# ishine/usdm

Measured on AMD Instinct MI355X. Metric: end-to-end real-time factor + LLM tokens/sec, 10 s utterance, 7B TP=1/8, higher is better.
Workload: dtype bf16; 1 GPU; full pipeline, one 10 s utterance: XLS-R tokenizer -> Mistral-7B (3 greedy rounds) -> Token-Voicebox 63 NFE (Heun, CFG, 3 s prompt) -> BigVGAN; wave_samples=160000, mel_frames=861, output_samples=220416, parallelism=tp1 (LLM) + replicas, tp_comm=none, voicebox=replica (CFG batch 2 on every rank)

## Files before the change

include/usdm_hip.h:

```cpp
#ifndef USDM_HIP_H_
#define USDM_HIP_H_
#include <stdint.h>

#ifdef __cplusplus
extern "C" {
#endif

typedef void* usdm_stream_t;

enum { USDM_BF16 = 0, USDM_F32 = 1 };
enum { USDM_ACT_NONE = 0, USDM_ACT_GELU = 1, USDM_ACT_SWIGLU = 3, USDM_ACT_TANH = 4, USDM_ACT_LOGCLAMP = 5  };
enum { USDM_EPI_PLAIN = 0, USDM_EPI_QKV_HEADS = 1 };

const char* usdm_last_error(void);
int usdm_abi_version(void);

typedef struct usdm_gemm_args {
  int32_t dtype;
  int32_t M, N;
  int32_t taps, Kc;
  const void* A;
  int64_t lda;
  int32_t rowsA;
  int32_t a_row_mul, a_row_off, a_row_step;
// ... 143 lines not shown
int64_t usdm_gemv_batch_ks_floats(int32_t N, int32_t K);
int usdm_gemv_batch(const usdm_gemv_batch_args* args, usdm_stream_t stream);

typedef struct usdm_gemv_fp8_args {
  usdm_gemv_batch_args b;
  const int8_t* row_exp;
} usdm_gemv_fp8_args;
int usdm_gemv_fp8(const usdm_gemv_fp8_args* args, usdm_stream_t stream);
int usdm_gemv_fp8_mfma(const usdm_gemv_fp8_args* args, usdm_stream_t stream);
int usdm_dequant_fp8(const void* q, const int8_t* row_exp, int32_t N, int32_t K, int64_t ldq, void* out, int64_t ldo,
                     usdm_stream_t stream);
int usdm_sizeof_gemv_fp8_args(void);

typedef struct usdm_gemv_mxfp4_args {
  usdm_gemv_batch_args b;
  const uint8_t* scales;
  int64_t lds;
} usdm_gemv_mxfp4_args;
int usdm_gemv_mxfp4(const usdm_gemv_mxfp4_args* args, usdm_stream_t stream);
int usdm_dequant_mxfp4(const void* codes, int64_t ldw, const uint8_t* scales, int64_t lds, int32_t N, int32_t K, void* out,
                       int64_t ldo, usdm_stream_t stream);
int usdm_sizeof_gemv_mxfp4_args(void);

typedef struct usdm_decode_state {
  int32_t* next_token;
  int32_t* out_tokens;
  int32_t* step;
  int32_t* pos;
  int32_t max_out, id_offset, advance_pos;
  int32_t batch;
  int32_t* done; const int32_t* eos;
} usdm_decode_state;
int usdm_argmax_final(const float* part_val, const int32_t* part_idx, int32_t nparts,
                      const usdm_decode_state* st, const void* embed_table_bf16, int32_t Hd, void* h_out_bf16,
                      usdm_stream_t stream);
int usdm_argmax_final_seg(const float* part_val, const int32_t* part_idx, int32_t nparts, int32_t nseg, int64_t seg_stride,
                          const usdm_decode_state* st, const void* embed_table, int32_t Hd, void* h_out, usdm_stream_t stream);

typedef struct usdm_sample_params {
  float temperature; int32_t top_k; float top_p;
  float min_p;
  uint64_t seed;
} usdm_sample_params;
typedef struct usdm_sample_args {
  const float* logits; int32_t V;
  float temperature; int32_t top_k; float top_p;
// ... 243 lines not shown
```

usdm_amd/_lib.py:

```python
import ctypes as C
import os

_HERE = os.path.dirname(os.path.abspath(__file__))
LIB_PATH = os.path.join(_HERE, "libusdm_hip.so")


class UsdmError(RuntimeError):
    pass


if not os.path.exists(LIB_PATH):
    raise ImportError(
        f"{LIB_PATH} not found: build it with `python -m usdm_amd.build` (hipcc --offload-arch=gfx950). "
        "usdm_amd has no CPU fallback.")

lib = C.CDLL(LIB_PATH, mode=C.RTLD_GLOBAL)
lib.usdm_last_error.restype = C.c_char_p
lib.usdm_gemv_batch_ks_floats.restype = C.c_int64
lib.usdm_gemv_fp8_mfma.restype = C.c_int
lib.usdm_attn_decode_fp8.restype = C.c_int
lib.usdm_rope_cache_fp8.restype = C.c_int
lib.usdm_gemv_mxfp4.restype = C.c_int
lib.usdm_dequant_mxfp4.restype = C.c_int
lib.usdm_logprobs.restype = C.c_int
lib.usdm_logprobs_seg.restype = C.c_int
lib.usdm_prompt_logprobs.restype = C.c_int
lib.usdm_prompt_logprobs_seg.restype = C.c_int
lib.usdm_penalize.restype = C.c_int
lib.usdm_penalize_seg.restype = C.c_int
lib.usdm_penalty_params_init.restype = C.c_int
lib.usdm_logit_edit.restype = C.c_int
lib.usdm_logit_edit_seg.restype = C.c_int
lib.usdm_beam_step.restype = C.c_int
lib.usdm_kv_reorder.restype = C.c_int
lib.usdm_kv_expand.restype = C.c_int
lib.usdm_attn_verify.restype = C.c_int
lib.usdm_spec_commit.restype = C.c_int
lib.usdm_attn_verify_batch.restype = C.c_int
lib.usdm_spec_commit_batch.restype = C.c_int
_exp = None


def exp():
    global _exp
    if _exp is None:
        path = os.path.join(_HERE, "libusdm_hip_experimental.so")
# ... 302 lines not shown
```

usdm_amd/csrc/gemv_common.h:

```cpp
#pragma once
#include "common.h"
#include "../../include/usdm_hip.h"

#ifndef USDM_UNR1
#define USDM_UNR1 8
#endif

namespace {
typedef __attribute__((ext_vector_type(2))) __bf16 bf16x2;

__device__ __forceinline__ float dot8(u32x4 w, u32x4 x, float acc) {
#pragma unroll
  for (int i = 0; i < 4; ++i) {
    const unsigned a = w[i], b = x[i];
    acc = __builtin_amdgcn_fdot2_f32_bf16(__builtin_bit_cast(bf16x2, a), __builtin_bit_cast(bf16x2, b), acc, false);
  }
  return acc;
}

template <bool FP8> struct gemv_fmt { typedef u32x4 wvec; };
template <> struct gemv_fmt<true> { typedef u32x2 wvec; };
struct gemv_mx4 { const uint8_t* scales; int64_t lds; };
template <class... FMT> struct gemv_is_mx4 { static constexpr bool value = false; };
template <> struct gemv_is_mx4<gemv_mx4> { static constexpr bool value = true; };
template <int I> struct gemv_ic { static constexpr int value = I; };
__device__ __forceinline__ const int8_t* gemv_row_exp() { return nullptr; }
__device__ __forceinline__ const int8_t* gemv_row_exp(const int8_t* e) { return e; }
__device__ __forceinline__ gemv_mx4 gemv_mx4_fmt() { return gemv_mx4{nullptr, 0}; }
__device__ __forceinline__ gemv_mx4 gemv_mx4_fmt(const int8_t*) { return gemv_mx4{nullptr, 0}; }
__device__ __forceinline__ gemv_mx4 gemv_mx4_fmt(gemv_mx4 m) { return m; }
constexpr int gemv_ring_depth(int NR, bool FP8, bool MX4) {
  const int bf16_depth = NR >= 8 ? 2 : NR >= 4 ? 4 : NR == 3 ? 5 : NR == 2 ? 8 : USDM_UNR1;
  return MX4 ? (NR >= 3 ? 2 : 4) : FP8 ? 2 * bf16_depth : bf16_depth;
}

__device__ __forceinline__ float gemv_sumsq8(u32x4 v, float ss) {
#pragma unroll
  for (int e = 0; e < 4; ++e) {
    const float lo = bf2f(v[e] & 0xffff), hi = bf2f(v[e] >> 16);
    ss += lo * lo + hi * hi;
  }
  return ss;
}
__device__ __forceinline__ u32x4 gemv_rmsnorm8(u32x4 v, float rstd, float4 g0, float4 g1) {
  const float gw[8] = {g0.x, g0.y, g0.z, g0.w, g1.x, g1.y, g1.z, g1.w};
  u32x4 o;
#pragma unroll
  for (int e = 0; e < 4; ++e) {
    const float lo = bf2f(v[e] & 0xffff), hi = bf2f(v[e] >> 16);
    o[e] = pack_bf2(round_bf(round_bf(lo * rstd) * gw[2 * e]), round_bf(round_bf(hi * rstd) * gw[2 * e + 1]));
  }
  return o;
}
__device__ __forceinline__ int gemv_glu_row(int o, bool up) { return (o >> 4) * 32 + (o & 15) + (up ? 16 : 0); }
__device__ __forceinline__ float gemv_swiglu_value(float g, float u, bool round_bf16) {
  if (round_bf16) {
// ... 17 lines not shown
```

usdm_amd/csrc/gemv_pieces.h:

```cpp
#pragma once
#include "gemv_common.h"

namespace {
__device__ __forceinline__ void gemv_load16(u32x4& dst, const void* p) {
  asm volatile("global_load_dwordx4 %0, %1, off" : "=v"(dst) : "v"(p) : "memory");
}
__device__ __forceinline__ void gemv_early_loads(const usdm_gemv_args& a, int i0, int K, u32x4& x0, u32x4& ge0v, u32x4& ge1v) {
  const int ic = min(i0, K - 8);
  const float* gp0 = a.norm_w ? a.norm_w + ic : (const float*)a.x;
  const float* gp1 = a.norm_w ? gp0 + 4 : gp0;
  gemv_load16(x0, (const bf16_t*)a.x + ic);
  gemv_load16(ge0v, gp0);
  gemv_load16(ge1v, gp1);
}
template <int IT>
__device__ __forceinline__ void gemv_ring_load(u32x4& dst, const char* row, unsigned voff) {
  const unsigned vo = voff + (IT >> 2) * 4096u;
  asm volatile("global_load_dwordx4 %0, %1, %2 offset:%3 nt" : "=v"(dst) : "v"(vo), "s"(row), "n"((IT & 3) * 1024) : "memory");
}

template <int NWV>
__device__ __forceinline__ float gemv_rms_rstd(float ss, float* red, int K, float eps) {
  const int lane = threadIdx.x & 63, wave = threadIdx.x >> 6;
  ss = wave_sum(ss);
  if (lane == 0) red[wave] = ss;
  __syncthreads();
  float tot = 0.f;
#pragma unroll
  for (int w = 0; w < NWV; ++w) tot += red[w];
  return rsqrtf(tot / (float)K + eps);
}
}
```

usdm_amd/csrc/llm_k.hip:

```cpp
#include "common.h"
#include <stdlib.h>
#include <utility>
#include "../../include/usdm_hip.h"
#include "gemv_launch.h"
#include "gemv_pieces.h"
#include "attn_merge.h"
#include "p2p.h"
#include "pick_commit.h"

#ifndef USDM_GEMV_DOWN_UNR
#define USDM_GEMV_DOWN_UNR 8
#endif
namespace {
#ifdef USDM_GEMV_TRACE
__device__ unsigned long long g_gemv_trace[8192 * 8];
#define GTR(i) do { if (threadIdx.x == 0 && blockIdx.x < 8192) g_gemv_trace[blockIdx.x * 8 + (i)] = wall_clock64(); } while (0)
#else
#define GTR(i) do { } while (0)
#endif


template <int RW, bool GLU, int NWV, bool MRG = false, bool P2P = false, bool CMB = false, bool FP8 = false, class... FMT>
__global__ __launch_bounds__(NWV * 64) void gemv_kernel(const usdm_gemv_args a, FMT... fmt) {
  typedef typename gemv_fmt<FP8>::wvec wvec;
  constexpr bool MX4 = gemv_is_mx4<FMT...>::value;
  static_assert((FP8 || MX4) == (sizeof...(FMT) == 1) && !(FP8 && MX4), "FP8 takes the row exponents, MXFP4 the block scales");
  static_assert(!(FP8 || MX4) || (!MRG && !P2P && !CMB), "the FP8 / MXFP4 weight formats have the plain single-GPU forms only");
  constexpr int NTH = NWV * 64;
  constexpr int NR = GLU ? 2 * RW : RW;
  constexpr int UNR = gemv_ring_depth(NR, FP8, MX4);
  extern __shared__ __attribute__((aligned(16))) char smem[];
  bf16_t* xs = (bf16_t*)smem;
  __shared__ float red[NWV];
  __shared__ float sv[NWV];
// ... 528 lines not shown
  __syncthreads();
  GTR(2);

  float acc = 0.f;
  u32x4 xv = *(const u32x4*)(xs + lane * 8);
  gemv_for<NIT>([&](auto IT) {
    constexpr int it = decltype(IT)::value, u = it % UNR;
    constexpr int younger = it + UNR < NIT ? UNR - 1 : NIT - 1 - it;
    const u32x4 xn = *(const u32x4*)(xs + (((it + 1) % NIT) * 64 + lane) * 8);
    asm volatile("s_waitcnt vmcnt(%1)" : "+v"(ring[u]) : "n"(younger) : "memory");
    acc = dot8(ring[u], xv, acc);
    if constexpr (it + UNR < NIT) gemv_ring_load<it + UNR>(ring[u], wp, voff);
    xv = xn;
  });
  acc = wave_sum(acc);
  GTR(3);

  if (lane != 0 || ob >= a.N) return;
  const float v = gemv_plain_value(acc, a.round_bf16, a.residual != nullptr, [&] { return bf2f(resraw); });
  if (a.y16) ((bf16_t*)a.y16)[ob] = f2bf(v);
  if (a.y32) a.y32[ob] = v;
}

__global__ void argmax_final_kernel(const float* pv, const int* pi, int nparts, int nseg, int64_t seg_stride, usdm_decode_state st,
                                    const bf16_t* E, int Hd, bf16_t* h_out) {
  __shared__ float sv[256];
  __shared__ int si[256];
  __shared__ int s_tok;
  const int b = blockIdx.x;
  if (st.done && st.done[b]) return;
  pv += (int64_t)b * nparts; pi += (int64_t)b * nparts;
  float bv = -INFINITY;
  int bi = PICK_NO_ID;
  for (int sg = 0; sg < nseg; ++sg)
    for (int i = threadIdx.x; i < nparts; i += 256) {
      const float v = pv[sg * seg_stride + i];
      const int id = pi[sg * seg_stride + i];
      if (pick_better(v, id, bv, bi)) { bv = v; bi = id; }
    }
  pick_block_best<256>(sv, si, bv, bi);
  if (threadIdx.x == 0) {
    const int tok = (si[0] == PICK_NO_ID ? 0 : si[0]) + st.id_offset;
    pick_commit(st, b, st.step[b], tok);
    s_tok = tok;
  }
  if (E) {
// ... 93 lines not shown
  USDM_CHECK_ARG(!a.x_out || (a.x_delta && a.x_out != a.x), "usdm_gemv: x_out needs x_delta and must not alias x");
  USDM_CHECK_ARG(!a.mrg_po || (a.mrg_pm && a.mrg_pl && a.mrg_ns >= 1 && a.mrg_ns <= 64 && a.K % 128 == 0 && !a.norm_w && !a.x_delta),
                 "usdm_gemv: merged-attention input needs pm/pl/po, 1 <= splits <= 64, K a multiple of 128, no norm / x_delta");
  USDM_CHECK_ARG(a.p2p_mode >= 0 && a.p2p_mode <= 2, "usdm_gemv: p2p_mode");
  USDM_CHECK_ARG(!a.p2p_mode || (a.p2p && a.p2p_site >= 0 && a.act == USDM_ACT_NONE && !a.part_val && a.residual && a.y16),
                 "usdm_gemv: the fused all-reduce needs a plain row-parallel projection with residual + y16");
  const int nout = glu ? a.N / 2 : a.N;
  hipStream_t st = (hipStream_t)stream;
  if (a.cmb_gran) {
    USDM_CHECK_ARG(a.mrg_po && a.mrg_pm && a.mrg_pl && a.mrg_ns >= 1 && a.mrg_ns <= 64 && !a.p2p_mode && !glu && !a.part_val && !a.norm_w && !a.x_delta &&
                       nout % 256 == 0 && nout / 256 == 16 && a.K % 128 == 0 && a.K / 128 <= 256,
                   "usdm_gemv: cmb_gran needs the mrg_* partials, a plain 4096-output projection and K / 128 <= 256 heads");
    return gemv_launch<GEMV_CMB, false, false, true, false>(a, st);
  }
  if (a.mrg_po || a.p2p_mode) {
    USDM_CHECK_ARG(!glu && !a.part_val, "usdm_gemv: merged-attention input / fused all-reduce are for plain projections");
    if (a.mrg_po && a.p2p_mode) return gemv_launch<GEMV_MRG, true, true, false, false>(a, st);
    if (a.mrg_po) return gemv_launch<GEMV_MRG, true, false, false, false>(a, st);
    return gemv_launch<GEMV_MRG, false, true, false, false>(a, st);
  }
  return gemv_launch<GEMV_PLAIN, false, false, false, false>(a, st);
}

int usdm_gemv_fp8_batch_launch(const usdm_gemv_fp8_args* pa, hipStream_t st);

extern "C" int usdm_gemv_fp8(const usdm_gemv_fp8_args* pa, usdm_stream_t stream) {
  USDM_CHECK_ARG(pa && pa->b.g.W && pa->b.g.x && pa->row_exp, "usdm_gemv_fp8: null args");
  const usdm_gemv_args& a = pa->b.g;
  USDM_CHECK_ARG(pa->b.nb >= 1 && pa->b.nb <= 4 && (pa->b.form == 0 || pa->b.form == -1),
                 "usdm_gemv_fp8: 1..4 sequences on the VALU form (the matrix-core form has no FP8 weights)");
  USDM_CHECK_ARG(!a.p2p && !a.p2p_mode && !a.mrg_po && !a.cmb_gran && !a.x_delta && !a.x_out,
                 "usdm_gemv_fp8: p2p / merged-attention input / cmb_gran / x_delta are not supported with FP8 weights");
  USDM_CHECK_ARG(((uintptr_t)a.W & 7) == 0, "usdm_gemv_fp8: bad N/K/ldw");
  if (int rc = gemv_check_shape("usdm_gemv_fp8", a, "input vector")) return rc;
  if (int rc = gemv_check_outputs("usdm_gemv_fp8", a)) return rc;
  hipStream_t st = (hipStream_t)stream;
  if (pa->b.nb > 1) return usdm_gemv_fp8_batch_launch(pa, st);
  return gemv_launch<GEMV_PLAIN, false, false, false, true>(a, st, pa->row_exp);
}

namespace {
__global__ __launch_bounds__(256) void dequant_fp8_kernel(const uint8_t* q, const int8_t* row_exp, int K, int64_t ldq, bf16_t* out,
                                                          int64_t ldo) {
  const int r = blockIdx.x;
  const float s = fp8_row_scale(row_exp[r]);
  const uint8_t* qr = q + (int64_t)r * ldq;
// ... 126 lines not shown
```

usdm_amd/llm.py:

```python
import math
import os
from collections import namedtuple

import torch

from . import ops
from ._lib import ACT_SWIGLU
from .graph import GraphedPlan, GraphedSegments
from .plancache import LRU
from .prefix import reusable_past
from .quant import Fp8Weight, Mxfp4Weight, check_kv_cache_dtype
from .slots import (CHUNK, NO_CANDIDATE_IDX, BeamSlots, DecodeSlots, SpecSequence, SpecSlots, TokenLogprobs, edit_buffers, logprob_buffers,
                    penalty_buffers, read_logprobs, seed_edits, seed_penalties, stop_block, stop_index)

MISTRAL_7B_USDM = dict(vocab_size=42003, hidden_size=4096, intermediate_size=14336, num_hidden_layers=32,
                       num_attention_heads=32, num_key_value_heads=8, head_dim=128, rms_norm_eps=1e-5,
                       rope_theta=10000.0, max_position_embeddings=32768)


def _pack_gate_up(gate, up):
    I, K = gate.shape
    return torch.stack([gate.reshape(I // 16, 16, K), up.reshape(I // 16, 16, K)], 1).reshape(2 * I, K).contiguous()


def vocab_shard(V, rank, tp):
    Vloc = (V + tp - 1) // tp
    v0 = min(V, rank * Vloc)
    v1 = min(V, v0 + Vloc)
    return Vloc, v0, v1, ops.gemv_nblocks(Vloc)


def agree_seed(seed, group, rank, device=None):
    import torch.distributed as dist
    if hasattr(group, "usdm_all_gather"):
# ... 122 lines not shown
    g = lambda n: sd_get(n).to(device, dtype)
    f = lambda n: sd_get(n).to(device, torch.float32).contiguous()
    W = {"embed": g("model.embed_tokens.weight").contiguous(), "norm": f("model.norm.weight"),
         "lm_head": qz_head(g("lm_head.weight")[v0:v1].contiguous()), "layers": [], "v0": v0, "v1": v1}
    for l in range(cfg["num_hidden_layers"]):
        p = f"model.layers.{l}."
        q = g(p + "self_attn.q_proj.weight")[rank * Hq * d:(rank + 1) * Hq * d]
        k = g(p + "self_attn.k_proj.weight")[rank * Hkv * d:(rank + 1) * Hkv * d]
        v = g(p + "self_attn.v_proj.weight")[rank * Hkv * d:(rank + 1) * Hkv * d]
        o = g(p + "self_attn.o_proj.weight")[:, rank * Hq * d:(rank + 1) * Hq * d]
        ga = g(p + "mlp.gate_proj.weight")[rank * I:(rank + 1) * I]
        up = g(p + "mlp.up_proj.weight")[rank * I:(rank + 1) * I]
        dn = g(p + "mlp.down_proj.weight")[:, rank * I:(rank + 1) * I]
        W["layers"].append(dict(qkv=qz(torch.cat([q, k, v], 0).contiguous()), o=qz(o.contiguous()), gu=qz(_pack_gate_up(ga, up)),
                                down=qz(dn.contiguous()), ln1=f(p + "input_layernorm.weight"),
                                ln2=f(p + "post_attention_layernorm.weight")))
        del q, k, v, o, ga, up, dn
    return W


class USDMForCausalLM:
    def __init__(self, cfg, device, ctx_max=2048, tp_rank=0, tp_size=1, group=None, decode_splits=None, tp_segments=None, p2p=None,
                 p2p_fused=None, quantization=None, fp8_matrix_cores=False, kv_cache_dtype=None, score_rows=256,
                 enable_prefix_caching=False):
        check_quantization(quantization, fp8_matrix_cores)
        self.prefix_caching = bool(enable_prefix_caching)
        if self.prefix_caching:
            if tp_size > 1 or tp_segments or p2p is not None:
                raise NotImplementedError("enable_prefix_caching runs on one GPU: tensor parallelism (tp_size > 1, tp_segments, p2p) is not supported")
            if os.environ.get("USDM_PREFIX_REUSE", "exact") in ("0", "off"):
                raise ValueError("enable_prefix_caching=True contradicts USDM_PREFIX_REUSE=0 (prefix reuse switched off)")
        if isinstance(score_rows, bool) or not isinstance(score_rows, int) or score_rows < 16 or score_rows % 16:
            raise ValueError(f"score_rows must be a positive multiple of 16, got {score_rows!r}")
        self.score_rows = score_rows
        if quantization is not None and (tp_size > 1 or tp_segments or p2p is not None):
            raise NotImplementedError(f"quantization={quantization!r} runs on one GPU: tensor parallelism (tp_size > 1, tp_segments, p2p) takes bf16 weights")
        self.kv_cache_dtype = check_kv_cache_dtype(kv_cache_dtype)
        self.kv8 = self.kv_cache_dtype == "fp8"
        if self.kv8 and (tp_size > 1 or tp_segments or p2p is not None):
            raise NotImplementedError("kv_cache_dtype='fp8' runs on one GPU: tensor parallelism (tp_size > 1, tp_segments, p2p) takes a bf16 cache")
        if self.kv8 and os.environ.get("USDM_GEMV_CHAIN", "0") not in ("", "0"):
            raise NotImplementedError("kv_cache_dtype='fp8': the chained decode GEMVs (USDM_GEMV_CHAIN) take a bf16 cache")
        self.quantization = quantization
        self.fp8_matrix_cores = bool(fp8_matrix_cores)
        self.cfg = dict(cfg)
        self.device = torch.device(device)
        if self.device.type != "cuda":
            raise RuntimeError("USDMForCausalLM (usdm_amd) runs on the MI355X only; there is no CPU fallback")
# ... 123 lines not shown
                           p + "self_attn.o_proj.weight": ((H, c["num_attention_heads"] * d), H ** -0.5),
                           p + "mlp.gate_proj.weight": ((I, H), H ** -0.5), p + "mlp.up_proj.weight": ((I, H), H ** -0.5),
                           p + "mlp.down_proj.weight": ((H, I), I ** -0.5)})

        def get(n):
            if n.endswith("norm.weight") or n.endswith("layernorm.weight"):
                return torch.ones(H, device=m.device)
            shape, sc = shapes[n]
            return (torch.randn(shape, device=m.device, dtype=torch.float32, generator=gen) * sc).to(torch.bfloat16)
        m.W = m._shard(get)
        m._alloc()
        return m

    def weight_bytes_per_token(self):
        if self.quantization is not None:
            return sum(l[k].nbytes for l in self.W["layers"] for k in QUANT_KEYS) + self.W["lm_head"].nbytes
        n = sum(l[k].numel() for l in self.W["layers"] for k in ("qkv", "o", "gu", "down")) + self.W["lm_head"].numel()
        return 2 * n

    def kv_bytes_per_token_row(self):
        d = self.cfg["head_dim"]
        return 2 * self.cfg["num_hidden_layers"] * self.Hkv * ((d + 1) if self.kv8 else 2 * d)

    def _alloc(self):
        c, dev = self.cfg, self.device
        L, d = c["num_hidden_layers"], c["head_dim"]
        bf = torch.bfloat16
        if self.kv8:
            self.kcache = torch.zeros(L, self.Hkv, self.ctx_max, d, dtype=torch.uint8, device=dev)
            self.vcache = torch.zeros(L, self.Hkv, self.ctx_max, d, dtype=torch.uint8, device=dev)
            self.kexp = torch.zeros(L, self.Hkv, self.ctx_max, dtype=torch.int8, device=dev)
            self.vexp = torch.zeros(L, self.Hkv, self.ctx_max, dtype=torch.int8, device=dev)
        else:
            self.kcache = torch.zeros(L, self.Hkv, self.ctx_max, d, dtype=bf, device=dev)
            self.vcache = torch.zeros(L, self.Hkv, self.ctx_max, d, dtype=bf, device=dev)
        mode = os.environ.get("USDM_PREFIX_REUSE", "exact")
        self.reuse_prefix = {"0": False, "off": False, "1": True, "all": True}.get(mode, "exact")
        if self.kv8:
            self.vtc = None
            if not self.prefix_caching:
                self.reuse_prefix = False
        else:
            self.vtc = torch.zeros(L, self.Hkv, d, self.ctx_max, dtype=bf, device=dev)
        self._kv_ids, self._vt_upto = None, 0
        inv_freq = 1.0 / (c["rope_theta"] ** (torch.arange(0, d, 2, dtype=torch.int64).float() / d))
        fr = torch.arange(self.ctx_max).float()[:, None] * inv_freq[None, :]
        self.cos = fr.cos().to(bf).to(dev).contiguous()
# ... 146 lines not shown
                ops.penalize(logits, st, V=self.v1 - self.v0, plan=rec.plan, **pen)
            if sampling == "hook":
                rec.cut(lambda: self.logits_hook())
            ops.sample_final(logits, st, dev_params=sl.sample_params, plan=rec.plan, **out)
            if lp:
                ops.logprobs(logits, st, V=self.v1 - self.v0, plan=rec.plan, **lp)
        elif p2p is not None:
            site = 2 * c["num_hidden_layers"]
            self._p2p_exchange(rec, st, lambda ph: ops.argmax_p2p(sl.part_val_loc, sl.part_idx_loc, self.nparts, st, p2p, site, phase=ph,
                                                                  plan=rec.plan, **out))
        else:
            if self.tp_path:
                rec.cut(self._gather_partials if single else
                        (lambda: self._gather_partials([sl.part_val, sl.part_idx], [sl.part_val_loc, sl.part_idx_loc])))
            seg = dict(nseg=self.tp_size, seg_stride=B * self.nparts) if (B and self.tp_path) else {}
            ops.argmax_final(sl.part_val, sl.part_idx, self.nparts * (1 if B else self.tp_size), st, plan=rec.plan, **seg, **out)
        rec.plan.hold(st)

    def _dims(self):
        c = self.cfg
        H, d = c["hidden_size"], c["head_dim"]
        return H, d, c["num_hidden_layers"], self.Hq, self.Hkv, self.I, (self.Hq + 2 * self.Hkv) * d

    def _layers(self, rec, gemv, attn, h, qkv, ao, act, way, n=0, parts=None, h_alt=None, down_kw={}):
        H, d, _, Hq, Hkv, I, nq = self._dims()
        eps, h0, pend = self.cfg["rms_norm_eps"], h, None

        def proj(W, ln, N, out, a=0):
            nonlocal h, pend
            if pend is None:
                return gemv(W, h, N=N, K=H, norm_w=ln, eps=eps, act=a, y16=out)
            nxt = h_alt if h is h0 else h0
            gemv(W, h, N=N, K=H, norm_w=ln, eps=eps, act=a, y16=out, x_delta=pend, x_out=nxt)
            h, pend = nxt, None

        def land(W, x, K, site, **kw):
            nonlocal pend
            if way == "fused":
                return gemv(W, x, N=H, K=K, residual=h, y16=h, **kw)
            if way == "p2p":
                mode = 1 if self.p2p_fused else 2
                gemv(W, x, N=H, K=K, residual=h, y16=h, p2p=self.p2p, p2p_site=site, p2p_mode=mode, **kw)
                rec.cut()
                if mode == 2:
                    ops.p2p_reduce(self.p2p, site, H, h, skip=self.st_done, plan=rec.plan)
                return
            part = parts[site & 1]
            gemv(W, x, N=H, K=K, round_bf16=False, y32=part, **kw)
            rec.cut(lambda: self._all_reduce(part))
            if way == "deferred":
                pend = part
            else:
                ops.residual_add(h, part, n, plan=rec.plan)

        for l, w in enumerate(self.W["layers"]):
            proj(w["qkv"], w["ln1"], nq, qkv)
            o_kw = attn(l) or {}
            land(w["o"], ao, Hq * d, 2 * l, **o_kw)
            proj(w["gu"], w["ln2"], 2 * I, act, ACT_SWIGLU)
            land(w["down"], act, I, 2 * l + 1, **down_kw)
        return h, pend

    def _prefill_rows(self, S, slot=None, past=0):
        dev, bf = self.device, torch.bfloat16
        H, d, L, Hq, Hkv, I, nq = self._dims()
        scratch = slot is not None or self.kv8
        Spad = ((past if scratch else 0) + S + 63) // 64 * 64
        rec = _Segments()
        Z = lambda *s, dt=bf: rec.plan.hold(torch.zeros(*s, device=dev, dtype=dt))
        io = dict(ids=Z(S, dt=torch.int64))
        h, xn, qkv, ao, act = Z(S, H), Z(S, H), Z(S, nq), Z(S, Hq * d), Z(S, I)
        vt = Z(Hkv, d, Spad) if scratch else None
        kscr = Z(Hkv, Spad, d) if self.kv8 else None
        part = Z(S, H, dt=torch.float32) if self.tp_path else None
        ops.embed_rows(self.W["embed"], h, Hd=H, ids=io["ids"], n=S, plan=rec.plan)

        def gemm(W, x, *, N, K, norm_w=None, eps=None, act=0, residual=None, y16=None, y32=None, round_bf16=True):
            if norm_w is not None:
                ops.norm(x, norm_w, None, rows=S, C=H, eps=eps, rms=True, round_bf16=True, out16=xn, plan=rec.plan)
                x = xn
            ops.gemm(x, self._gemm_w(W, rec.plan), M=S, N=N, Kc=K, act=act, round_bf16=round_bf16 and (bool(act) or residual is not None),
                     residual=residual, ldr=H if residual is not None else 0, out32=y32, out16=y16, ldc=N // 2 if act else N, plan=rec.plan)

# ... 95 lines not shown
                ops.gemv_engine(chain, sync, self.chain_gran, plan=rec.plan)
            else:
                ops.gemv_chain(chain, sync, plan=rec.plan)
            chain = None

        def gemv(W, x, **kw):
            if chain is None:
                return ops.gemv(W, x, skip=skp, plan=rec.plan, **kw)
            chain.append(ops.gemv(W, x, skip=skp, only_args=True, **kw))
            if len(chain) == self.chain:
                flush()

        def attn(l):
            nonlocal chain
            gran = cmb_gran[l] if use_cmb else None
            ops.attn_decode(qkv, self.st_pos, self.cos, self.sin, self.kcache[l], self.vcache[l], pm, pl, po, ao, Hq=Hq, Hkv=Hkv,
                            ctx_max=self.ctx_max, NS=self.NS, scale=d ** -0.5, counters=cnt, skip=skp, defer_merge=mrg is not None, window=self.window,
                            cmb_gran=gran, kv8=(self.kexp[l], self.vexp[l]) if self.kv8 else None, plan=rec.plan)
            if chained:
                chain = []
                return None
            return dict(merge=mrg, cmb=(gran, self.cmb_err) if use_cmb else None)

        h, pend = self._layers(rec, gemv, attn, h, qkv, ao, act, way, n=H, parts=parts, h_alt=h_alt)
        if chain:
            flush()
        self._lm_head_and_pick(rec, h, True, sampling, x_delta=pend, skip=skp, logprobs=logprobs, penalties=penalties, edits=edits)
        return rec.finish()

    @staticmethod
    def _run_segs(segs):
        for s in segs:
            if isinstance(s, ops.Plan):
                s.run()
            else:
                s()

    def _graphed(self, built, enabled=None):
        segs = built if isinstance(built, list) else [built]
        if any(not isinstance(s, ops.Plan) for s in segs):
            return GraphedSegments(segs, self._run_segs, enabled=enabled)
        plan = segs[0]
        if len(segs) > 1:
            plan = ops.Plan()
            for s in segs:
                plan.calls += s.calls
                plan.hold(*s.keep)
# ... 504 lines not shown
```

usdm_amd/ops.py:

```python
import ctypes as C_
import os

import torch

from . import _lib
from ._lib import (BF16, F32, AttnVerifyArgs, AttnVerifyBatchArgs, SpecArgs, SpecBatchArgs, BeamArgs, KvExpandArgs, KvReorderArgs, AttnArgs, AttnDecodeArgs, AttnDecodeFp8Args, RopeFp8Args, DecodeState, GemmArgs, GemvArgs, GemvBatchArgs, GemvFp8Args, GemvMxfp4Args, LogitEditArgs, LogprobArgs, NormArgs, PenaltyArgs, PromptLogprobArgs, RopeArgs, SampleArgs, SnakeArgs,
                   VbInputArgs, VbSolverArgs, check, lib)
from .quant import Fp8Weight, Mxfp4Weight


def _stream():
    return C_.c_void_p(torch.cuda.current_stream().cuda_stream)


class Plan:

    def __init__(self):
        self.calls = []
        self.keep = []

    def add(self, what, fn, *args):
        self.calls.append((what, fn, args))

    def hold(self, *tensors):
        self.keep.extend(tensors)
        return tensors[0] if len(tensors) == 1 else tensors

    def run(self):
        st = _stream()
        for what, fn, args in self.calls:
            rc = fn(*args, st)
# ... 181 lines not shown
    n = units.numel()
    nframes = (n * rep) // hop
    out = torch.empty(nframes, dtype=torch.int64, device=units.device)
    if n == 0 or nframes == 0:
        return out
    check(lib.usdm_process_unit(_ptr(units.contiguous()), C_.c_int32(n), C_.c_int32(rep), C_.c_int32(hop), _ptr(out),
                                C_.c_int32(nframes), _stream()), "usdm_process_unit")
    return out


def _fill_gemv(a, W, x, *, N, K, ldw=None, norm_w=None, eps=1e-5, act=0, round_bf16=True, residual=None, y16=None, y32=None,
               ban=None, part_val=None, part_idx=None, idx_offset=0):
    _need_cuda(W, x, norm_w, residual, y16, y32, ban, part_val, part_idx)
    a.W, a.ldw, a.N, a.K = _ptr(W), (ldw if ldw is not None else K), N, K
    if isinstance(W, Mxfp4Weight):
        a.ldw = W.q.shape[1]
    a.x, a.norm_w, a.eps = _ptr(x), _ptr(norm_w), eps
    a.act, a.round_bf16 = act, int(round_bf16)
    a.residual, a.y16, a.y32 = _ptr(residual), _ptr(y16), _ptr(y32)
    a.ban, a.part_val, a.part_idx, a.idx_offset = _ptr(ban), _ptr(part_val), _ptr(part_idx), idx_offset


def gemv(W, x, *, x_delta=None, x_out=None, skip=None, p2p=None, p2p_site=0, p2p_mode=0, merge=None, cmb=None, plan=None,
         only_args=False, resident=None, **common):
    _need_cuda(x_delta, x_out, skip)
    if x_out is not None and x_out.data_ptr() == x.data_ptr():
        raise ValueError("usdm_gemv: x_out must not alias x")
    a = GemvArgs()
    _fill_gemv(a, W, x, **common)
    a.x_delta, a.x_out, a.skip = _ptr(x_delta), _ptr(x_out), _ptr(skip)
    if resident is None:
        resident = int(os.environ.get("USDM_GEMV_RESIDENT", "0"))
    a.resident = resident
    if merge is not None:
        pm, pl, po, ns = merge
        _need_cuda(pm, pl, po)
        a.mrg_pm, a.mrg_pl, a.mrg_po, a.mrg_ns = _ptr(pm), _ptr(pl), _ptr(po), ns
    if cmb is not None:
        gran, err = cmb
        _need_cuda(gran, err)
        if merge is None or gran.numel() * gran.element_size() < (a.K // 2) * 8:
            raise ValueError("usdm_gemv: cmb needs merge=(pm, pl, po, NS) and K/2 8-byte granules")
        a.cmb_gran, a.cmb_err, a.cmb_timeout_ms = _ptr(gran), _ptr(err), 200
    if p2p is not None and p2p_mode:
        p2p.check_site(p2p_site, a.N)
        a.p2p, a.p2p_site, a.p2p_mode = p2p.dev_ptr, p2p_site, p2p_mode
    if isinstance(W, Fp8Weight):
        if only_args:
            raise ValueError("usdm_gemv: FP8 weights have no chained form")
        f = GemvFp8Args()
        f.b.g, f.b.nb, f.row_exp = a, 1, _ptr(W.e)
        _go(plan, "usdm_gemv_fp8", lib.usdm_gemv_fp8, C_.byref(f))
        return
    if isinstance(W, Mxfp4Weight):
        if only_args:
            raise ValueError("usdm_gemv: MXFP4 weights have no chained form")
        f = GemvMxfp4Args()
        f.b.g, f.b.nb, f.scales, f.lds = a, 1, _ptr(W.s), W.s.shape[1]
        _go(plan, "usdm_gemv_mxfp4", lib.usdm_gemv_mxfp4, C_.byref(f))
        return
    if only_args:
        return a
    _go(plan, "usdm_gemv", lib.usdm_gemv, C_.byref(a))


def gemv_engine(phases, sync, gran, timeout_ms=2000, plan=None):
    _need_cuda(sync, gran)
    if not (1 <= len(phases) <= 4) or sync.numel() < 8 or sync.element_size() != 4 or gran.numel() * gran.element_size() < 3 * 8192 * 8:
        raise ValueError("gemv_engine: 1..4 phases, an 8-word sync block and 192 KB of granule space")
    c = _lib.GemvChainArgs()
    for i, ph in enumerate(phases):
        c.ph[i] = ph
    c.nph, c.sync, c.timeout_ms, c.gran = len(phases), _ptr(sync), timeout_ms, _ptr(gran)
    _go(plan, "usdm_gemv_engine", _lib.exp().usdm_gemv_engine, C_.byref(c))


def gemv_chain(phases, sync, timeout_ms=2000, plan=None):
    _need_cuda(sync)
    if not (1 <= len(phases) <= 4) or sync.numel() < 8 or sync.element_size() != 4:
        raise ValueError("gemv_chain: 1..4 phases and an 8-word sync block")
    c = _lib.GemvChainArgs()
    for i, ph in enumerate(phases):
# ... 538 lines not shown
```

Baseline: 5.398 x real-time (output audio s / wall s).

## Stream down-projection weights from a lossless exponent-packed image in decode GEMV

Adds a load-time packer that stores each bf16 weight of the MLP down projection as its low byte, a 4-bit exponent offset from a matrix-wide base, and a sign bit. That is 3328 bytes per 2048 weights instead of 4096. A new GEMV kernel rebuilds the bf16 values in registers with byte permutes. Rows whose exponents fall outside the 16-value window keep the original bf16 streaming path. The goal is to cut HBM bytes read by the memory-bound decode GEMV. The cost is extra device memory for the packed image, decode ALU work, and little gain if many rows end up marked.

New measurement: 5.524 x real-time (output audio s / wall s), median of 6. +2.3%, better.

```diff
diff --git a/include/usdm_hip.h b/include/usdm_hip.h
--- a/include/usdm_hip.h
+++ b/include/usdm_hip.h
@@ -189,6 +189,18 @@
                        int64_t ldo, usdm_stream_t stream);
 int usdm_sizeof_gemv_mxfp4_args(void);
 
+typedef struct usdm_gemv_wpack {
+  const void* planes;
+  const uint8_t* rowflag;
+  int64_t stride;
+  int32_t base;
+  int32_t units;
+  uint32_t marked[448];
+} usdm_gemv_wpack;
+int usdm_gemv_packed(const usdm_gemv_args* args, const usdm_gemv_wpack* pack, usdm_stream_t stream);
+int usdm_gemv_packs(const usdm_gemv_args* args);
+int usdm_sizeof_gemv_wpack(void);
+
 typedef struct usdm_decode_state {
   int32_t* next_token;
   int32_t* out_tokens;
diff --git a/usdm_amd/_lib.py b/usdm_amd/_lib.py
--- a/usdm_amd/_lib.py
+++ b/usdm_amd/_lib.py
@@ -22,6 +22,8 @@
 lib.usdm_rope_cache_fp8.restype = C.c_int
 lib.usdm_gemv_mxfp4.restype = C.c_int
 lib.usdm_dequant_mxfp4.restype = C.c_int
+lib.usdm_gemv_packed.restype = C.c_int
+lib.usdm_gemv_packs.restype = C.c_int
 lib.usdm_logprobs.restype = C.c_int
 lib.usdm_logprobs_seg.restype = C.c_int
 lib.usdm_prompt_logprobs.restype = C.c_int
diff --git a/usdm_amd/csrc/gemv_common.h b/usdm_amd/csrc/gemv_common.h
--- a/usdm_amd/csrc/gemv_common.h
+++ b/usdm_amd/csrc/gemv_common.h
@@ -32,6 +32,19 @@
 constexpr int gemv_ring_depth(int NR, bool FP8, bool MX4) {
   const int bf16_depth = NR >= 8 ? 2 : NR >= 4 ? 4 : NR == 3 ? 5 : NR == 2 ? 8 : USDM_UNR1;
   return MX4 ? (NR >= 3 ? 2 : 4) : FP8 ? 2 * bf16_depth : bf16_depth;
+}
+
+constexpr unsigned GEMV_WPACK_UNIT = 3328;
+template <int P>
+__device__ __forceinline__ u32x4 gemv_wpack8(unsigned lo0, unsigned lo1, unsigned nib, unsigned sgn, unsigned base4) {
+  const unsigned h0 = ((nib & 0x0f0f0f0fu) + base4) | ((sgn << (2 * P)) & 0x80808080u);
+  const unsigned h1 = (((nib >> 4) & 0x0f0f0f0fu) + base4) | ((sgn << (2 * P + 1)) & 0x80808080u);
+  u32x4 w;
+  w[0] = __builtin_amdgcn_perm(h0, lo0, 0x05010400u);
+  w[1] = __builtin_amdgcn_perm(h0, lo0, 0x07030602u);
+  w[2] = __builtin_amdgcn_perm(h1, lo1, 0x05010400u);
+  w[3] = __builtin_amdgcn_perm(h1, lo1, 0x07030602u);
+  return w;
 }
 
 __device__ __forceinline__ float gemv_sumsq8(u32x4 v, float ss) {
diff --git a/usdm_amd/csrc/gemv_pieces.h b/usdm_amd/csrc/gemv_pieces.h
--- a/usdm_amd/csrc/gemv_pieces.h
+++ b/usdm_amd/csrc/gemv_pieces.h
@@ -18,6 +18,15 @@
   const unsigned vo = voff + (IT >> 2) * 4096u;
   asm volatile("global_load_dwordx4 %0, %1, %2 offset:%3 nt" : "=v"(dst) : "v"(vo), "s"(row), "n"((IT & 3) * 1024) : "memory");
 }
+struct gemv_wunit { u32x4 la, lb, nib; unsigned sgn; };
+template <int U>
+__device__ __forceinline__ void gemv_unit_load(gemv_wunit& d, const char* row, unsigned voff) {
+  const unsigned vo = voff + U * GEMV_WPACK_UNIT, vs = (voff >> 2) + U * GEMV_WPACK_UNIT;
+  asm volatile("global_load_dwordx4 %0, %1, %2 nt" : "=v"(d.la) : "v"(vo), "s"(row) : "memory");
+  asm volatile("global_load_dwordx4 %0, %1, %2 offset:1024 nt" : "=v"(d.lb) : "v"(vo), "s"(row) : "memory");
+  asm volatile("global_load_dwordx4 %0, %1, %2 offset:2048 nt" : "=v"(d.nib) : "v"(vo), "s"(row) : "memory");
+  asm volatile("global_load_dword %0, %1, %2 offset:3072 nt" : "=v"(d.sgn) : "v"(vs), "s"(row) : "memory");
+}
 
 template <int NWV>
 __device__ __forceinline__ float gemv_rms_rstd(float ss, float* red, int K, float eps) {
diff --git a/usdm_amd/csrc/llm_k.hip b/usdm_amd/csrc/llm_k.hip
--- a/usdm_amd/csrc/llm_k.hip
+++ b/usdm_amd/csrc/llm_k.hip
@@ -10,6 +10,12 @@
 
 #ifndef USDM_GEMV_DOWN_UNR
 #define USDM_GEMV_DOWN_UNR 8
+#endif
+#ifndef USDM_GEMV_WPACK_RU
+#define USDM_GEMV_WPACK_RU 3
+#endif
+#ifndef USDM_GEMV_WPACK_UB
+#define USDM_GEMV_WPACK_UB 12
 #endif
 namespace {
 #ifdef USDM_GEMV_TRACE
@@ -584,6 +590,84 @@
   if (a.y32) a.y32[ob] = v;
 }
 
+template <int NIT, int RU, int UB>
+__global__ __launch_bounds__(1024) __attribute__((amdgpu_waves_per_eu(4))) void gemv_stream_wpack_kernel(const usdm_gemv_args a,
+                                                                                                        const usdm_gemv_wpack p) {
+  constexpr int NWV = 16, NTH = NWV * 64, K = NIT * 512, NU = NIT / 4;
+  static_assert(NIT % 4 == 0 && NU >= RU && RU >= 1 && NIT >= UB && UB >= 1 && K <= 2 * NTH * 8, "whole units; a full first ring");
+  extern __shared__ __attribute__((aligned(16))) char smem[];
+  bf16_t* xs = (bf16_t*)smem;
+  const int tid = threadIdx.x, lane = tid & 63, wave = tid >> 6;
+  int skipv = a.skip ? *a.skip : 0;
+  const int ob = blockIdx.x * NWV + wave;
+  const int urow = min((int)blockIdx.x * NWV + __builtin_amdgcn_readfirstlane(wave), a.N - 1);
+  const bool marked = (p.marked[urow >> 5] >> (urow & 31)) & 1u;
+  const unsigned voff = lane * 16;
+  const bf16_t* rbase = a.residual ? (const bf16_t*)a.residual : (const bf16_t*)a.W;
+  const unsigned short resraw = rbase[min(ob, a.N - 1)];
+  const int i0 = tid * 8, i1 = i0 + NTH * 8;
+  const bf16_t* xp0 = (const bf16_t*)a.x + min(i0, K - 8);
+  const bf16_t* xp1 = (const bf16_t*)a.x + min(i1, K - 8);
+  float acc = 0.f;
+  if (marked) {
+    const char* wp = (const char*)((const bf16_t*)a.W + (int64_t)urow * a.ldw);
+    u32x4 x0, x1;
+    gemv_load16(x0, xp0);
+    gemv_load16(x1, xp1);
+    u32x4 ring[UB];
+    gemv_for<UB>([&](auto U) { gemv_ring_load<U.value>(ring[U.value], wp, voff); });
+    asm volatile("s_waitcnt vmcnt(%3)" : "+v"(x0), "+v"(x1), "+s"(skipv) : "n"(UB));
+    if (skipv) return;
+    if (i0 < K) *(u32x4*)(xs + i0) = x0;
+    if (i1 < K) *(u32x4*)(xs + i1) = x1;
+    __syncthreads();
+    u32x4 xv = *(const u32x4*)(xs + lane * 8);
+    gemv_for<NIT>([&](auto IT) {
+      constexpr int it = decltype(IT)::value, u = it % UB;
+      constexpr int younger = it + UB < NIT ? UB - 1 : NIT - 1 - it;
+      const u32x4 xn = *(const u32x4*)(xs + (((it + 1) % NIT) * 64 + lane) * 8);
+      asm volatile("s_waitcnt vmcnt(%1)" : "+v"(ring[u]) : "n"(younger) : "memory");
+      acc = dot8(ring[u], xv, acc);
+      if constexpr (it + UB < NIT) gemv_ring_load<it + UB>(ring[u], wp, voff);
+      xv = xn;
+    });
+  } else {
+    const char* pp = (const char*)p.planes + (int64_t)urow * p.stride;
+    const unsigned base4 = (unsigned)p.base * 0x01010101u;
+    u32x4 x0, x1;
+    gemv_load16(x0, xp0);
+    gemv_load16(x1, xp1);
+    gemv_wunit ring[RU];
+    gemv_for<RU>([&](auto U) { gemv_unit_load<U.value>(ring[U.value], pp, voff); });
+    asm volatile("s_waitcnt vmcnt(%3)" : "+v"(x0), "+v"(x1), "+s"(skipv) : "n"(4 * RU));
+    if (skipv) return;
+    if (i0 < K) *(u32x4*)(xs + i0) = x0;
+    if (i1 < K) *(u32x4*)(xs + i1) = x1;
+    __syncthreads();
+    u32x4 xv = *(const u32x4*)(xs + lane * 8);
+    gemv_for<NU>([&](auto UI) {
+      constexpr int un = decltype(UI)::value, s = un % RU;
+      constexpr int younger = un + RU < NU ? 4 * (RU - 1) : 4 * (NU - 1 - un);
+      gemv_wunit& r = ring[s];
+      asm volatile("s_waitcnt vmcnt(%4)" : "+v"(r.la), "+v"(r.lb), "+v"(r.nib), "+v"(r.sgn) : "n"(younger) : "memory");
+      gemv_for<4>([&](auto PI) {
+        constexpr int P = decltype(PI)::value, it = 4 * un + P;
+        const u32x4 xn = *(const u32x4*)(xs + (((it + 1) % NIT) * 64 + lane) * 8);
+        const u32x4& lo = P < 2 ? r.la : r.lb;
+        acc = dot8(gemv_wpack8<P>(lo[2 * (P & 1)], lo[2 * (P & 1) + 1], r.nib[P], r.sgn, base4), xv, acc);
+        xv = xn;
+      });
+      if constexpr (un + RU < NU) gemv_unit_load<un + RU>(r, pp, voff);
+    });
+  }
+  acc = wave_sum(acc);
+
+  if (lane != 0 || ob >= a.N) return;
+  const float v = gemv_plain_value(acc, a.round_bf16, a.residual != nullptr, [&] { return bf2f(resraw); });
+  if (a.y16) ((bf16_t*)a.y16)[ob] = f2bf(v);
+  if (a.y32) a.y32[ob] = v;
+}
+
 __global__ void argmax_final_kernel(const float* pv, const int* pi, int nparts, int nseg, int64_t seg_stride, usdm_decode_state st,
                                     const bf16_t* E, int Hd, bf16_t* h_out) {
   __shared__ float sv[256];
@@ -723,6 +807,27 @@
   return gemv_launch<GEMV_PLAIN, false, false, false, false>(a, st);
 }
 
+extern "C" int usdm_gemv_packs(const usdm_gemv_args* pa) { return gemv_select(*pa, false).stream ? 1 : 0; }
+
+extern "C" int usdm_gemv_packed(const usdm_gemv_args* pa, const usdm_gemv_wpack* pk, usdm_stream_t stream) {
+  USDM_CHECK_ARG(pa && pa->W && pa->x && pk && pk->planes && pk->rowflag, "usdm_gemv_packed: null args");
+  USDM_CHECK_ARG(pa->N <= 14336, "usdm_gemv_packed: at most 14336 rows (usdm_gemv_wpack.marked)");
+  if (!usdm_gemv_packs(pa)) return usdm_gemv(pa, stream);
+  const usdm_gemv_args& a = *pa;
+  if (int rc = gemv_check_shape("usdm_gemv_packed", a, "input vector")) return rc;
+  if (int rc = gemv_check_outputs("usdm_gemv_packed", a)) return rc;
+  USDM_CHECK_ARG(pk->units == 7 && pk->units * 2048 == a.K && pk->stride % 16 == 0 && pk->stride >= (int64_t)pk->units * GEMV_WPACK_UNIT &&
+                     pk->base >= 0 && pk->base <= 112,
+                 "usdm_gemv_packed: the image must hold K / 2048 units of 3328 bytes per row, stride a multiple of 16, base 0..112");
+  USDM_CHECK_ARG(((uintptr_t)pk->planes & 15) == 0 && ((uintptr_t)pk->rowflag & 3) == 0, "usdm_gemv_packed: planes must be 16-byte, rowflag 4-byte aligned");
+  const gemv_sel s = gemv_select(a, false);
+  hipLaunchKernelGGL((gemv_stream_wpack_kernel<28, USDM_GEMV_WPACK_RU, USDM_GEMV_WPACK_UB>), dim3(s.grid), dim3(1024), (size_t)a.K * 2,
+                     (hipStream_t)stream, a, *pk);
+  USDM_LAUNCH_CHECK();
+  return 0;
+}
+extern "C" int usdm_sizeof_gemv_wpack(void) { return (int)sizeof(usdm_gemv_wpack); }
+
 int usdm_gemv_fp8_batch_launch(const usdm_gemv_fp8_args* pa, hipStream_t st);
 
 extern "C" int usdm_gemv_fp8(const usdm_gemv_fp8_args* pa, usdm_stream_t stream) {
diff --git a/usdm_amd/llm.py b/usdm_amd/llm.py
--- a/usdm_amd/llm.py
+++ b/usdm_amd/llm.py
@@ -1,5 +1,6 @@
 import math
 import os
+import time
 from collections import namedtuple
 
 import torch
@@ -10,6 +11,7 @@
 from .plancache import LRU
 from .prefix import reusable_past
 from .quant import Fp8Weight, Mxfp4Weight, check_kv_cache_dtype
+from .wpack import PackedWeight
 from .slots import (CHUNK, NO_CANDIDATE_IDX, BeamSlots, DecodeSlots, SpecSequence, SpecSlots, TokenLogprobs, edit_buffers, logprob_buffers,
                     penalty_buffers, read_logprobs, seed_edits, seed_penalties, stop_block, stop_index)
 
@@ -178,8 +180,10 @@
 class USDMForCausalLM:
     def __init__(self, cfg, device, ctx_max=2048, tp_rank=0, tp_size=1, group=None, decode_splits=None, tp_segments=None, p2p=None,
                  p2p_fused=None, quantization=None, fp8_matrix_cores=False, kv_cache_dtype=None, score_rows=256,
-                 enable_prefix_caching=False):
+                 enable_prefix_caching=False, weight_packing=None):
         check_quantization(quantization, fp8_matrix_cores)
+        self.weight_packing = (os.environ.get("USDM_WPACK", "1") != "0") if weight_packing is None else bool(weight_packing)
+        self.wpack_report = None
         self.prefix_caching = bool(enable_prefix_caching)
         if self.prefix_caching:
             if tp_size > 1 or tp_segments or p2p is not None:
@@ -349,7 +353,20 @@
         d = self.cfg["head_dim"]
         return 2 * self.cfg["num_hidden_layers"] * self.Hkv * ((d + 1) if self.kv8 else 2 * d)
 
+    def _pack_weights(self):
+        self.wpack_down = None
+        if not (self.weight_packing and self.tp_size == 1 and not self.tp_path and self.p2p is None and self.quantization is None
+                and self.cfg["hidden_size"] == 4096 and self.I == 14336):
+            return
+        t0 = time.perf_counter()
+        self.wpack_down = [PackedWeight.from_matrix(w["down"]) for w in self.W["layers"]]
+        torch.cuda.synchronize(self.device)
+        self.wpack_report = {"down_marked_share": [p.marked_share for p in self.wpack_down],
+                             "down_marked_rows": sum(len(p.marked_rows) for p in self.wpack_down),
+                             "extra_bytes": sum(p.nbytes for p in self.wpack_down), "seconds": time.perf_counter() - t0}
+
     def _alloc(self):
+        self._pack_weights()
         c, dev = self.cfg, self.device
         L, d = c["num_hidden_layers"], c["head_dim"]
         bf = torch.bfloat16
@@ -542,7 +559,7 @@
         H, d = c["hidden_size"], c["head_dim"]
         return H, d, c["num_hidden_layers"], self.Hq, self.Hkv, self.I, (self.Hq + 2 * self.Hkv) * d
 
-    def _layers(self, rec, gemv, attn, h, qkv, ao, act, way, n=0, parts=None, h_alt=None, down_kw={}):
+    def _layers(self, rec, gemv, attn, h, qkv, ao, act, way, n=0, parts=None, h_alt=None, down_kw={}, down_wp=None):
         H, d, _, Hq, Hkv, I, nq = self._dims()
         eps, h0, pend = self.cfg["rms_norm_eps"], h, None
 
@@ -578,7 +595,7 @@
             o_kw = attn(l) or {}
             land(w["o"], ao, Hq * d, 2 * l, **o_kw)
             proj(w["gu"], w["ln2"], 2 * I, act, ACT_SWIGLU)
-            land(w["down"], act, I, 2 * l + 1, **down_kw)
+            land(w["down"], act, I, 2 * l + 1, **down_kw, **({"wpack": down_wp[l]} if down_wp else {}))
         return h, pend
 
     def _prefill_rows(self, S, slot=None, past=0):
@@ -720,7 +737,8 @@
                 return None
             return dict(merge=mrg, cmb=(gran, self.cmb_err) if use_cmb else None)
 
-        h, pend = self._layers(rec, gemv, attn, h, qkv, ao, act, way, n=H, parts=parts, h_alt=h_alt)
+        h, pend = self._layers(rec, gemv, attn, h, qkv, ao, act, way, n=H, parts=parts, h_alt=h_alt,
+                               down_wp=self.wpack_down if way == "fused" else None)
         if chain:
             flush()
         self._lm_head_and_pick(rec, h, True, sampling, x_delta=pend, skip=skp, logprobs=logprobs, penalties=penalties, edits=edits)
diff --git a/usdm_amd/ops.py b/usdm_amd/ops.py
--- a/usdm_amd/ops.py
+++ b/usdm_amd/ops.py
@@ -7,6 +7,10 @@
 from ._lib import (BF16, F32, AttnVerifyArgs, AttnVerifyBatchArgs, SpecArgs, SpecBatchArgs, BeamArgs, KvExpandArgs, KvReorderArgs, AttnArgs, AttnDecodeArgs, AttnDecodeFp8Args, RopeFp8Args, DecodeState, GemmArgs, GemvArgs, GemvBatchArgs, GemvFp8Args, GemvMxfp4Args, LogitEditArgs, LogprobArgs, NormArgs, PenaltyArgs, PromptLogprobArgs, RopeArgs, SampleArgs, SnakeArgs,
                    VbInputArgs, VbSolverArgs, check, lib)
 from .quant import Fp8Weight, Mxfp4Weight
+from .wpack import GemvWpack
+
+if lib.usdm_sizeof_gemv_wpack() != C_.sizeof(GemvWpack):
+    raise ImportError(f"ABI mismatch: usdm_gemv_wpack is {lib.usdm_sizeof_gemv_wpack()} bytes in the library, {C_.sizeof(GemvWpack)} in Python")
 
 
 def _stream():
@@ -234,7 +238,7 @@
 
 
 def gemv(W, x, *, x_delta=None, x_out=None, skip=None, p2p=None, p2p_site=0, p2p_mode=0, merge=None, cmb=None, plan=None,
-         only_args=False, resident=None, **common):
+         only_args=False, resident=None, wpack=None, **common):
     _need_cuda(x_delta, x_out, skip)
     if x_out is not None and x_out.data_ptr() == x.data_ptr():
         raise ValueError("usdm_gemv: x_out must not alias x")
@@ -270,6 +274,14 @@
         f = GemvMxfp4Args()
         f.b.g, f.b.nb, f.scales, f.lds = a, 1, _ptr(W.s), W.s.shape[1]
         _go(plan, "usdm_gemv_mxfp4", lib.usdm_gemv_mxfp4, C_.byref(f))
+        return
+    if wpack is not None and not only_args and lib.usdm_gemv_packs(C_.byref(a)):
+        if not wpack.is_cuda or (wpack.N, wpack.K) != (a.N, a.K):
+            raise ValueError("usdm_gemv: wpack is the image of another matrix")
+        p = wpack.args()
+        if plan is not None:
+            plan.hold(wpack.planes, wpack.rowflag)
+        _go(plan, "usdm_gemv", lib.usdm_gemv_packed, C_.byref(a), C_.byref(p))
         return
     if only_args:
         return a
diff --git a/usdm_amd/wpack.py b/usdm_amd/wpack.py
--- /dev/null
+++ b/usdm_amd/wpack.py
@@ -0,0 +1,105 @@
+import ctypes as C
+
+import torch
+
+UNIT_ELEMS = 2048
+UNIT_BYTES = 3328
+MAX_ROWS = 14336
+
+
+def _i16(w):
+    if w.dtype != torch.bfloat16 or w.dim() != 2 or w.shape[1] % UNIT_ELEMS:
+        raise ValueError("wpack: a bf16 [N][K] matrix with K a multiple of 2048")
+    return w.contiguous().view(torch.int16).to(torch.int32) & 0xffff
+
+
+def _pick_base(e7):
+    rmin, rmax = e7.amin(dim=1), e7.amax(dim=1)
+    cand = torch.arange(0, 0x7f - 15 + 1, device=e7.device)
+    fits = ((rmin[None, :] >= cand[:, None]) & (rmax[None, :] <= cand[:, None] + 15)).sum(dim=1)
+    best = int(fits.max().item())
+    return int(cand[fits == best].min().item())
+
+
+def pack(w):
+    b = _i16(w)
+    N, K = b.shape
+    U = K // UNIT_ELEMS
+    e7 = (b >> 8) & 0x7f
+    base = _pick_base(e7)
+    idx = e7 - base
+    marked = ((idx < 0) | (idx > 15)).any(dim=1)
+    idx = idx & 15
+    v = lambda t: t.view(N, U, 4, 64, 8)
+    lo, ix, sg = v(b & 0xff), v(idx), v(b >> 15)
+    low = lo.permute(0, 1, 3, 2, 4).reshape(N, U, 64, 32)
+    la, lb = low[..., :16].reshape(N, U, 1024), low[..., 16:].reshape(N, U, 1024)
+    nib = (ix[..., :4] | (ix[..., 4:] << 4)).permute(0, 1, 3, 2, 4).reshape(N, U, 1024)
+    i_ = torch.arange(4, device=w.device).view(4, 1, 1)
+    k_ = torch.arange(8, device=w.device).view(1, 1, 8)
+    sh = 8 * (k_ & 3) + 7 - (2 * i_ + (k_ >> 2))
+    sd = (sg.to(torch.int64) << sh).sum(dim=(2, 4))
+    sb = torch.stack([(sd >> (8 * j)) & 0xff for j in range(4)], dim=-1).reshape(N, U, 256)
+    planes = torch.cat((la, lb, nib, sb.to(torch.int32)), dim=2).to(torch.uint8).reshape(N, U * UNIT_BYTES).contiguous()
+    flag = torch.zeros((N + 3) // 4 * 4, dtype=torch.uint8, device=w.device)
+    flag[:N] = marked.to(torch.uint8)
+    return planes, flag, base
+
+
+def unpack(planes, base, K):
+    N, U = planes.shape[0], K // UNIT_ELEMS
+    p = planes.view(N, U, UNIT_BYTES).to(torch.int32)
+    low = torch.cat((p[..., :1024].reshape(N, U, 64, 16), p[..., 1024:2048].reshape(N, U, 64, 16)), dim=3)
+    lo = low.view(N, U, 64, 4, 8).permute(0, 1, 3, 2, 4)
+    nb = p[..., 2048:3072].reshape(N, U, 64, 4, 4).permute(0, 1, 3, 2, 4)
+    ix = torch.cat((nb & 15, nb >> 4), dim=4)
+    sb = p[..., 3072:].reshape(N, U, 64, 4).to(torch.int64)
+    sd = (sb[..., 0] | (sb[..., 1] << 8) | (sb[..., 2] << 16) | (sb[..., 3] << 24)).view(N, U, 1, 64, 1)
+    i_ = torch.arange(4, device=planes.device).view(4, 1, 1)
+    k_ = torch.arange(8, device=planes.device).view(1, 1, 8)
+    sg = ((sd >> (8 * (k_ & 3) + 7 - (2 * i_ + (k_ >> 2)))) & 1).to(torch.int32)
+    return (lo | ((ix + base) << 8) | (sg << 15)).reshape(N, K)
+
+
+class GemvWpack(C.Structure):
+    _fields_ = [("planes", C.c_void_p), ("rowflag", C.c_void_p), ("stride", C.c_int64), ("base", C.c_int32), ("units", C.c_int32),
+                ("marked", C.c_uint32 * (MAX_ROWS // 32))]
+
+
+class PackedWeight:
+    __slots__ = ("planes", "rowflag", "base", "N", "K", "marked_rows")
+
+    def __init__(self, planes, rowflag, base, K):
+        self.planes, self.rowflag, self.base, self.K = planes, rowflag, int(base), K
+        self.N = planes.shape[0]
+        if self.N > MAX_ROWS:
+            raise ValueError(f"wpack: at most {MAX_ROWS} rows")
+        self.marked_rows = torch.nonzero(rowflag[:self.N]).flatten().tolist()
+
+    @classmethod
+    def from_matrix(cls, w):
+        planes, flag, base = pack(w)
+        ok = (unpack(planes, base, w.shape[1]) == _i16(w)).all(dim=1) | (flag[:w.shape[0]] != 0)
+        if not bool(ok.all()):
+            raise RuntimeError("wpack: the packed image does not reproduce the matrix")
+        return cls(planes, flag, base, w.shape[1])
+
+    @property
+    def is_cuda(self):
+        return self.planes.is_cuda
+
+    @property
+    def marked_share(self):
+        return len(self.marked_rows) / self.N
+
+    @property
+    def nbytes(self):
+        return self.planes.numel() + self.rowflag.numel()
+
+    def args(self):
+        a = GemvWpack()
+        a.planes, a.rowflag = C.c_void_p(self.planes.data_ptr()), C.c_void_p(self.rowflag.data_ptr())
+        a.stride, a.base, a.units = self.planes.shape[1], self.base, self.K // UNIT_ELEMS
+        for r in self.marked_rows:
+            a.marked[r >> 5] |= 1 << (r & 31)
+        return a
```
